# kisasexypantera94/hpfw

Measured on AMD Instinct MI355X. Metric: hashprints/sec (index) + Hamming matches/sec (search), 30 s@44.1 kHz clips, higher is better.
Workload: dtype f32 (transforms, dB) + int8 digits / int64 sums (projection); 1 GPU; configs[1]: 1000 x 30 s synthetic 44.1 kHz PCM16 clips per GPU, hashprint extraction only (CQT + dB + projection + bit pack), inputs resident in HBM; clips_per_gpu=1000, hashprints_per_clip=2320, parallelism=clips sharded over 1 GPU(s), no collective on this path

## Files before the change

hpfw_amd/csrc/extract.hip:

```cpp
#include "handle.h"

int pass_clips(hpfw_gpu *h, const DevPlan *dp, int64_t n_clips)
{
    const hpfw::HostPlan &p = dp->hp;
    size_t per_clip = (size_t)121 * p.c * 4 + (size_t)64 * std::max(p.n_frames, 1) * 4;
    if (p.bluestein)
        per_clip += 2 * hpfw::bz_plane_bytes(dp->bz, 1) + (size_t)(p.kmax - p.kmin) * 8;
    else
        per_clip += (size_t)hpfw::z_floats_per_clip(p.hq, p.n2) * 4 + (size_t)p.n1 * p.q2w * 8;
    size_t work = 0;
    for (const hpfw::CqClassDev &cd : dp->cls) work = std::max(work, hpfw::cq_big_work_bytes(cd, 1));
    per_clip += work;
    const int64_t fit = std::max<int64_t>(1, (int64_t)(((size_t)24 << 30) / per_clip));
    const int64_t cap = std::min<int64_t>(h->batch, fit), n = std::max<int64_t>(n_clips, 1);
    const int64_t passes = (n + cap - 1) / cap;
    return (int)((n + passes - 1) / passes);
}

int ensure_ws(hpfw_gpu *h, const DevPlan *dp, int nb, int ns)
{
    const hpfw::HostPlan &p = dp->hp;
    size_t work = 0;
    for (const hpfw::CqClassDev &cd : dp->cls) work = std::max(work, hpfw::cq_big_work_bytes(cd, nb));
    if (work) {
        int rc = ensure(h->d_cqwork, work);
        if (rc) return rc;
    }
    const size_t planar = p.bluestein ? hpfw::bz_plane_bytes(dp->bz, nb) : 0;
    const size_t need[7] = {p.bluestein ? planar : (size_t)nb * hpfw::z_floats_per_clip(p.hq, p.n2) * 4,
                            p.bluestein ? (size_t)nb * (p.kmax - p.kmin) * 8 : (size_t)nb * p.n1 * p.q2w * 8,
                            (size_t)ns * 121 * p.c * 4, (size_t)ns * 64 * (size_t)std::max(p.n_frames, 1) * 4,
                            (size_t)ns * 121 * hpfw::kCqMaxWaves * 4,
                            0, planar};
    for (int i = 0; i < 7; ++i) {
        int rc = ensure(h->ws[i], need[i], h);
        if (rc) return rc;
    }
    return ensure(h->d_clipmax, (size_t)ns * 4, h);
}

namespace {
int ensure_side_streams(hpfw_gpu *h)
{
    if (h->cq_join[hpfw_gpu::kCqSide - 1]) return HPFW_OK;
    bool ok = h->cq_fork.create() == hipSuccess;
    for (int k = 0; k < hpfw_gpu::kCqSide && ok; ++k) ok = h->cq_side[k].create() == hipSuccess && h->cq_join[k].create() == hipSuccess;
    return ok ? HPFW_OK : fail(HPFW_E_HIP, "side streams");
}

class Fanout {
public:
    Fanout(hpfw_gpu *h, hipStream_t s) : h_(h), s_(s) {}
    Fanout(const Fanout &) = delete;
    Fanout &operator=(const Fanout &) = delete;
    ~Fanout()
    {
        for (int k = 0; k < hpfw_gpu::kCqSide; ++k) {
            if (!(used_ >> k & 1u)) continue;
            hipStream_t side = h_->cq_side[k].get();
            hipEvent_t join = h_->cq_join[k].get();
            if (report(h_, hipEventRecord(join, side), "side stream join") || report(h_, hipStreamWaitEvent(s_, join, 0), "side stream join"))
                (void)hipStreamSynchronize(side);
        }
    }
    int fork(int n)
    {
        int rc = ensure_side_streams(h_);
        if (rc) return rc;
        HIP_TRY(hipEventRecord(h_->cq_fork.get(), s_));
        for (int k = 0; k < n; ++k) HIP_TRY(hipStreamWaitEvent(h_->cq_side[k].get(), h_->cq_fork.get(), 0));
        return 0;
    }
    hipStream_t lane(int k)
    {
        if (k == 0) return s_;
        used_ |= 1u << (k - 1);
        return h_->cq_side[k - 1].get();
    }

private:
    hpfw_gpu *h_;
    hipStream_t s_;
    unsigned used_ = 0;
};

#if defined(HPFW_ROWS_SNAP) || defined(HPFW_ROWS_STAMPS)
hpfw::cf *g_rows_snap = nullptr;
#endif

int run_forward(hpfw_gpu *h, DevPlan *dp, const int16_t *d_pcm, int nb, hpfw::cf *x, hipStream_t s)
{
    const hpfw::HostPlan &p = dp->hp;
    float *yp = h->ws[0].as<float>();
    int rc;
    if (p.bluestein) {
        float *other = h->ws[6].as<float>();
        if (h->bz_chunk > 0 && nb >= 6 * h->bz_chunk) {
            const int lanes = h->fwd_streams;
            Fanout fan(h, s);
            if (lanes > 1 && (rc = fan.fork(lanes - 1))) return rc;
            const int64_t region = (int64_t)(hpfw::bz_plane_bytes(dp->bz, h->bz_chunk) / sizeof(float));
            int i = 0;
            for (int c0 = 0; c0 < nb; c0 += h->bz_chunk, ++i) {
                const int nc = std::min(nb - c0, h->bz_chunk);
                const int lane = i % lanes;
                hipStream_t st = fan.lane(lane);
                float *ya = yp + lane * region, *yb = other + lane * region;
                {
                    Timed t(h, K_COLS, st);
                    hpfw::launch_bz_cols_first(dp->bz, d_pcm + (int64_t)c0 * p.n, p.n, nc, ya, st);
                }
                {
                    Timed t(h, K_ROWS, st);
                    hpfw::launch_bz_rows_both(dp->rows, dp->bz, ya, nc, yb, st);
                }
                {
                    Timed t(h, K_COLS, st);
                    hpfw::launch_bz_cols_last(dp->bz, yb, nc, x + (int64_t)c0 * dp->cq.xclip, st);
                }
            }
            return check_launch("bz_chunks");
        }
        {
            Timed t(h, K_COLS, s);
            hpfw::launch_bz_cols_first(dp->bz, d_pcm, p.n, nb, yp, s);
        }
        if ((rc = check_launch("bz_cols"))) return rc;
        {
            Timed t(h, K_ROWS, s);
            hpfw::launch_bz_rows_both(dp->rows, dp->bz, yp, nb, other, s);
        }
        if ((rc = check_launch("bz_rows"))) return rc;
        {
            Timed t(h, K_COLS, s);
            hpfw::launch_bz_cols_last(dp->bz, other, nb, x, s);
        }
        return check_launch("bz_cols");
    }
    Timed span(h, K_FWD, s);
    hpfw::ColsQArgs cols = dp->cols;
    cols.variant = h->cols_variant;
    if (h->fwd_chunk > 0 && nb >= 6 * h->fwd_chunk) {
        const int lanes = h->fwd_streams;
        Fanout fan(h, s);
        if (lanes > 1 && (rc = fan.fork(lanes - 1))) return rc;
        const int64_t region = (int64_t)h->fwd_chunk * dp->rows_out.zclip;
        int i = 0;
        for (int c0 = 0; c0 < nb; c0 += h->fwd_chunk, ++i) {
            const int nc = std::min(nb - c0, h->fwd_chunk);
            const int lane = i % lanes;
            hipStream_t st = fan.lane(lane);
            float *zr = yp + lane * region;
            {
                Timed t(h, K_COLS, st);
                hpfw::launch_fwd_cols_q(cols, d_pcm + (int64_t)c0 * p.n, p.n, nc, zr, st);
            }
            {
                Timed t(h, K_ROWS, st);
                hpfw::launch_fwd_rows2(dp->rows, dp->rows_out, zr, nc, x + (int64_t)c0 * dp->rows_out.n1 * dp->rows_out.q2w, st);
            }
        }
        return check_launch("fwd_chunks");
    }
    {
        Timed t(h, K_COLS, s);
        hpfw::launch_fwd_cols_q(cols, d_pcm, p.n, nb, yp, s);
    }
    if ((rc = check_launch("fwd_cols"))) return rc;
    {
        Timed t(h, K_ROWS, s);
#if defined(HPFW_ROWS_SNAP)
        dp->rows.snap = g_rows_snap;
#endif
#if defined(HPFW_ROWS_STAMPS)
        dp->rows.stamps = reinterpret_cast<long long *>(g_rows_snap);
#endif
        hpfw::launch_fwd_rows2(dp->rows, dp->rows_out, yp, nb, x, s);
    }
    return check_launch("fwd_rows");
}
}

int run_front(hpfw_gpu *h, DevPlan *dp, const int16_t *d_pcm, int nb, int slot, bool finish_db, hipStream_t s)
{
    using hpfw::cf;
    const hpfw::HostPlan &p = dp->hp;
    cf *x = h->ws[1].as<cf>();
    float *mag = h->ws[2].as<float>() + (size_t)slot * 121 * p.c;
    float *mm = h->ws[4].as<float>() + (size_t)slot * 121 * hpfw::kCqMaxWaves;
    float *clipmax = h->d_clipmax.as<float>() + slot;
    int rc;
    if ((rc = run_forward(h, dp, d_pcm, nb, x, s))) return rc;
    {
        Timed t(h, K_CQ, s);
        int n_lds = 0;
        for (const hpfw::CqClassDev &cd : dp->cls) n_lds += cd.outer ? 0 : 1;
        const bool fork = h->cq_concurrent && n_lds > 1 && nb >= 4;
        Fanout fan(h, s);
        if (fork && (rc = fan.fork(hpfw_gpu::kCqSide))) return rc;
        int turn = 0;
        for (size_t ci = dp->cls.size(); ci-- > 0;) {
            const hpfw::CqClassDev &cd = dp->cls[ci];
            if (cd.outer) {
                hpfw::launch_cq_big_class(dp->cq, cd, x, nb, h->d_cqwork.as<cf>(), mag, mm, h->db_fast ? hpfw::kDbFast : hpfw::kDbSpec, s);
                continue;
            }
            const int lane = fork ? turn++ % (hpfw_gpu::kCqSide + 1) : 0;
            hpfw::launch_cq_class(dp->cq, cd, x, nb, mag, mm, h->db_fast ? hpfw::kDbFast : hpfw::kDbSpec, fan.lane(lane));
        }
        if ((rc = check_launch("cq_chirpz"))) return rc;
    }
    {
        Timed t(h, K_DB, s);
        hpfw::launch_clipmax(mm, clipmax, nb, s);
        if (finish_db) hpfw::launch_db_finish(mag, clipmax, nb, (int64_t)121 * p.c, s);
    }
    return check_launch("db");
}

int q_split(hpfw_gpu *h, int n_shifts, int64_t n_clips, int64_t c, hpfw::QSplit *qs, const hpfw::QSplit **use)
{
    *use = nullptr;
    if (n_shifts || h->q_products != 6 || !h->projection) return 0;
    const int64_t tiles = hpfw::project_q_tiles(n_clips, c);
    if (tiles <= 0) return 0;
    if (int rc = ensure(h->d_q_split, hpfw::project_q_split_bytes(tiles), h)) return rc;
    *qs = {h->d_q_thr.as<int32_t>(), h->d_q_split.get()};
    *use = qs;
    return 0;
}

namespace {
int run_back(hpfw_gpu *h, DevPlan *dp, const void *images, int n_shifts, int ns, uint64_t *d_hp, hipStream_t s)
{
    const hpfw::HostPlan &p = dp->hp;
    const float *sdb = h->ws[2].as<float>();
    int rc;
    if (h->projection) {
        hpfw::QSplit qs;
        const hpfw::QSplit *split;
        if ((rc = q_split(h, n_shifts, ns, p.c, &qs, &split))) return rc;
        {
            Timed t(h, K_PROJECT, s);
            hpfw::launch_hashprints_q(images, n_shifts, sdb, h->d_clipmax.as<float>(), ns, p.c, d_hp, nullptr, s, split);
        }
        if (split) h->q_last_tiles = hpfw::project_q_tiles(ns, p.c);
        return check_launch("project");
    }
    float *proj = h->ws[3].as<float>();
    {
        Timed t(h, K_PROJECT, s);
        hpfw::launch_project(h->d_fpack.as<float>(), sdb, h->d_clipmax.as<float>(), ns, p.c, proj, s);
    }
    if ((rc = check_launch("project"))) return rc;
    {
        Timed t(h, K_PACK, s);
        hpfw::launch_pack(proj, ns, p.n_frames, d_hp, s);
    }
    return check_launch("delta_pack");
}

constexpr int kBackBatch = 1024;

int check_filters(const hpfw_gpu *h) { return h->has_filters ? 0 : fail(HPFW_E_NOFILTERS, "no filters: call hpfw_gpu_set_filters or hpfw_gpu_learn_filters first"); }

int check_shifts(const int32_t *shifts, int n_shifts)
{
    if (!shifts || n_shifts < 1 || n_shifts > hpfw::kMaxShifts) return fail(HPFW_E_INVALID, "shifts: 1 to 64 values");
    for (int i = 0; i < n_shifts; ++i) {
        if (shifts[i] < -(hpfw::kBins - 1) || shifts[i] > hpfw::kBins - 1) return fail(HPFW_E_INVALID, "shifts: |s| <= 120");
        for (int j = 0; j < i; ++j)
            if (shifts[j] == shifts[i]) return fail(HPFW_E_INVALID, "shifts: values must be distinct");
    }
    return 0;
}

int shift_images(hpfw_gpu *h, const int32_t *shifts, int n_shifts, hipStream_t s)
{
    std::vector<int32_t> want(shifts, shifts + n_shifts);
    if (want == h->shift_images_of) return 0;
    h->shift_images_of.clear();
    int rc;
    if ((rc = ensure(h->d_shift_images, (size_t)n_shifts * hpfw::project_q_image_bytes()))) return rc;
    hpfw::ShiftList sl{n_shifts, {}};
    for (int i = 0; i < n_shifts; ++i) sl.s[i] = shifts[i];
    hpfw::launch_shift_filter_images(h->d_fq_image.get(), sl, h->d_shift_images.get(), s);
    if ((rc = check_launch("shift_filter_images"))) return rc;
    h->shift_images_of = std::move(want);
    return 0;
}

int check_transposed(hpfw_gpu *h, const int32_t *shifts, int n_shifts)
{
    int rc;
    if ((rc = check_shifts(shifts, n_shifts))) return rc;
    if (!h) return fail(HPFW_E_INVALID, "null handle");
    if (!h->projection) return fail(HPFW_E_INVALID, "transposed extraction needs projection mode 1 (fixed point)");
    if ((rc = check_filters(h))) return rc;
    return 0;
}

int hashprints_from_db(hpfw_gpu *h, const float *d_db, int64_t n_clips, int64_t c, const int32_t *shifts, int n_shifts, uint64_t *d_hp,
                       hipStream_t s)
{
    const int64_t nf = c - (hpfw::kCtx - 1), nhp = nf - hpfw::kLag;
    HIP_TRY(hipSetDevice(h->device));
    return ordered_call(h, s, [&] {
        int rc;
        if (n_shifts && (rc = shift_images(h, shifts, n_shifts, s))) return rc;
        const void *images = n_shifts ? h->d_shift_images.get() : h->d_fq_image.get();
        const int nbmax = 256;
        if (!h->projection && (rc = ensure(h->ws[3], (size_t)nbmax * 64 * (size_t)nf * 4))) return rc;
        hpfw::QSplit qs;
        const hpfw::QSplit *split;
        if ((rc = q_split(h, n_shifts, std::min<int64_t>(nbmax, n_clips), c, &qs, &split))) return rc;
        for (int64_t c0 = 0; c0 < n_clips; c0 += nbmax) {
            const int nb = (int)std::min<int64_t>(nbmax, n_clips - c0);
            if (h->projection) {
                Timed t(h, K_PROJECT, s);
                hpfw::launch_hashprints_q(images, n_shifts, d_db + c0 * 121 * c, nullptr, nb, (int)c, d_hp + c0 * std::max(n_shifts, 1) * nhp,
                                          nullptr, s, split);
                if (split) h->q_last_tiles = hpfw::project_q_tiles(nb, c);
            } else {
                hpfw::launch_project(h->d_fpack.as<float>(), d_db + c0 * 121 * c, nullptr, nb, (int)c, h->ws[3].as<float>(), s);
                hpfw::launch_pack(h->ws[3].as<float>(), nb, (int)nf, d_hp + c0 * nhp, s);
            }
            if ((rc = check_launch("project"))) return rc;
        }
        return 0;
    });
}

constexpr size_t kTempoBudget = (size_t)256 << 20;

int check_tempos(const float *tempos, int n_tempos, int n_shifts)
{
    if (!tempos || n_tempos < 1 || n_tempos > hpfw::kMaxTempos) return fail(HPFW_E_INVALID, "tempos: 1 to 64 values");
    for (int i = 0; i < n_tempos; ++i) {
        if (!(tempos[i] >= 0.5f && tempos[i] <= 2.0f)) return fail(HPFW_E_INVALID, "tempos: finite values in [0.5, 2]");
        for (int j = 0; j < i; ++j)
            if (hpfw::tempo_step(tempos[j]) == hpfw::tempo_step(tempos[i]))
                return fail(HPFW_E_INVALID, "tempos: values must have distinct steps rint(65536 / tempo)");
    }
    if ((int64_t)n_tempos * std::max(n_shifts, 1) > hpfw::kMaxShifts) return fail(HPFW_E_INVALID, "tempos x shifts: at most 64 variants");
    return 0;
}

int check_tempo_call(hpfw_gpu *h, const float *tempos, int n_tempos, const int32_t *shifts, int n_shifts, hpfw::TempoList *tl)
{
    int rc;
    if ((rc = check_tempos(tempos, n_tempos, n_shifts))) return rc;
    if ((shifts || n_shifts) && (rc = check_shifts(shifts, n_shifts))) return rc;
    if (!h) return fail(HPFW_E_INVALID, "null handle");
    if (!h->projection) return fail(HPFW_E_INVALID, "tempo extraction needs projection mode 1 (fixed point)");
    if ((rc = check_filters(h))) return rc;
    tl->n = n_tempos;
    for (int i = 0; i < n_tempos; ++i) tl->step[i] = hpfw::tempo_step(tempos[i]);
    return 0;
}

int64_t tempo_common_columns(int64_t c, const hpfw::TempoList &tl)
{
    int64_t ct = INT64_MAX;
    for (int i = 0; i < tl.n; ++i) ct = std::min(ct, hpfw::tempo_columns(c, tl.step[i]));
    return ct;
}

int tempo_back(hpfw_gpu *h, const void *images, int n_shifts, const float *d_db, int64_t nb, int64_t c, const hpfw::TempoList &tl,
               int64_t ct, uint64_t *d_hp, hipStream_t s)
{
    const int64_t per_pair = (int64_t)std::max(n_shifts, 1) * (ct - (hpfw::kCtx - 1) - hpfw::kLag);
    const size_t pair_bytes = (size_t)hpfw::kBins * ct * 4;
    const int64_t pairs = std::max<int64_t>(1, (int64_t)(kTempoBudget / pair_bytes));
    const int64_t cb = pairs >= tl.n ? std::min<int64_t>(pairs / tl.n, nb) : 1;
    const int tb = pairs >= tl.n ? tl.n : (int)pairs;
    int rc;
    if ((rc = ensure(h->d_tempo, (size_t)cb * tb * pair_bytes, h))) return rc;
    float *scaled = h->d_tempo.as<float>();
    for (int64_t c0 = 0; c0 < nb; c0 += cb) {
        const int nc = (int)std::min(cb, nb - c0);
        for (int j0 = 0; j0 < tl.n; j0 += tb) {
            hpfw::TempoList sub{std::min(tb, tl.n - j0), {}};
            for (int j = 0; j < sub.n; ++j) sub.step[j] = tl.step[j0 + j];
            hpfw::launch_tempo_scale(d_db + c0 * hpfw::kBins * c, nc, c, sub, ct, scaled, s);
            if ((rc = check_launch("tempo_scale"))) return rc;
            {
                Timed t(h, K_PROJECT, s);
                hpfw::launch_hashprints_q(images, n_shifts, scaled, nullptr, nc * sub.n, (int)ct, d_hp + (c0 * tl.n + j0) * per_pair, nullptr, s);
            }
            if ((rc = check_launch("project"))) return rc;
        }
    }
    return 0;
}

int extract_tempo_pcm16(hpfw_gpu *h, const int16_t *d_pcm, int64_t n_samples, int64_t n_clips, const float *tempos, int n_tempos,
                        const int32_t *shifts, int n_shifts, uint64_t *d_hp, void *stream)
{
    hpfw::TempoList tl;
    int rc = check_tempo_call(h, tempos, n_tempos, shifts, n_shifts, &tl);
    if (rc) return rc;
    if (!d_pcm || !d_hp || n_clips < 0) return fail(HPFW_E_INVALID, "bad argument");
    HIP_TRY(hipSetDevice(h->device));
    DevPlan *dp;
    if ((rc = get_plan(h, n_samples, &dp))) return rc;
    const int64_t c = dp->hp.c, ct = tempo_common_columns(c, tl);
    if (ct - (hpfw::kCtx - 1) - hpfw::kLag < 1) return fail(HPFW_E_UNSUPPORTED, "clip too short to yield a hashprint at the slowest tempo");
    if (n_clips == 0) return 0;
    const int64_t per_clip = (int64_t)tl.n * std::max(n_shifts, 1) * (ct - (hpfw::kCtx - 1) - hpfw::kLag);
    hipStream_t s = (hipStream_t)stream;
    return ordered_call(h, s, [&] {
        if (n_shifts && (rc = shift_images(h, shifts, n_shifts, s))) return rc;
        const void *images = n_shifts ? h->d_shift_images.get() : h->d_fq_image.get();
        const int nbmax = pass_clips(h, dp, n_clips);
        if ((rc = ensure_ws(h, dp, nbmax, nbmax))) return rc;
        for (int64_t c0 = 0; c0 < n_clips; c0 += nbmax) {
            const int nb = (int)std::min<int64_t>(nbmax, n_clips - c0);
            if ((rc = run_front(h, dp, d_pcm + c0 * n_samples, nb, 0, true, s))) return rc;
            if ((rc = tempo_back(h, images, n_shifts, h->ws[2].as<float>(), nb, c, tl, ct, d_hp + c0 * per_clip, s))) return rc;
        }
        return 0;
    });
}

int extract_pcm16(hpfw_gpu *h, const int16_t *d_pcm, int64_t n_samples, int64_t n_clips, const int32_t *shifts, int n_shifts,
                  uint64_t *d_hp, void *stream)
{
    if (!h || !d_pcm || !d_hp || n_clips < 0) return fail(HPFW_E_INVALID, "bad argument");
    if (int rc = check_filters(h)) return rc;
    HIP_TRY(hipSetDevice(h->device));
    DevPlan *dp;
    int rc = get_plan(h, n_samples, &dp);
    if (rc) return rc;
    if (dp->hp.n_hp <= 0) return fail(HPFW_E_UNSUPPORTED, "clip too short to yield a hashprint");
    hipStream_t s = (hipStream_t)stream;
    return ordered_call(h, s, [&] {
        if (n_shifts && (rc = shift_images(h, shifts, n_shifts, s))) return rc;
        const void *images = n_shifts ? h->d_shift_images.get() : h->d_fq_image.get();
        const int nbmax = pass_clips(h, dp, n_clips);
        const int nsmax = (int)std::min<int64_t>(std::max(kBackBatch, nbmax), std::max<int64_t>(n_clips, 1));
        if ((rc = ensure_ws(h, dp, nbmax, nsmax))) return rc;
        for (int64_t s0 = 0; s0 < n_clips; s0 += nsmax) {
            const int ns = (int)std::min<int64_t>(nsmax, n_clips - s0);
            for (int c0 = 0; c0 < ns; c0 += nbmax) {
                const int nb = std::min(nbmax, ns - c0);
                if ((rc = run_front(h, dp, d_pcm + (s0 + c0) * n_samples, nb, c0, false, s))) return rc;
            }
            if ((rc = run_back(h, dp, images, n_shifts, ns, d_hp + s0 * std::max(n_shifts, 1) * dp->hp.n_hp, s))) return rc;
        }
        return 0;
    });
}

template <class Device>
int staged_pcm16_host(hpfw_gpu *h, const int16_t *pcm, int64_t n_samples, int64_t n_clips, int64_t per_clip, uint64_t *hp,
                      Device device)
{
    int rc;
    const int64_t chunk = std::min<int64_t>(n_clips, std::max<int64_t>(1, (192ll << 20) / (n_samples * 2)));
    if ((rc = ensure(h->stage_hp, (size_t)n_clips * std::max<int64_t>(per_clip, 1) * 8))) return rc;
    for (int b = 0; b < 2; ++b) {
        if (b == 1 && chunk >= n_clips) break;
        if ((rc = ensure(h->stage_pcm[b], (size_t)chunk * n_samples * 2))) return rc;
    }
    if (!h->stage_consumed[1]) {
        HIP_TRY(h->stage_copy.create());
        HIP_TRY(h->stage_comp.create());
        for (int b = 0; b < 2; ++b) {
            HIP_TRY(h->stage_copied[b].create());
            HIP_TRY(h->stage_consumed[b].create());
        }
    }
    hipStream_t s_copy = h->stage_copy.get(), s_comp = h->stage_comp.get();
    uint64_t *d_hp = h->stage_hp.as<uint64_t>();
    int64_t ci = 0;
    for (int64_t c0 = 0; !rc && c0 < n_clips; c0 += chunk, ++ci) {
        const int b = (int)(ci & 1);
        const int64_t cnt = std::min(chunk, n_clips - c0);
        int16_t *d_pcm = h->stage_pcm[b].as<int16_t>();
        hipEvent_t copied = h->stage_copied[b].get(), consumed = h->stage_consumed[b].get();
        if (ci >= 2 && hipStreamWaitEvent(s_copy, consumed, 0) != hipSuccess) rc = fail(HPFW_E_HIP, "event wait failed");
        if (!rc && hipMemcpyAsync(d_pcm, pcm + c0 * n_samples, (size_t)cnt * n_samples * 2, hipMemcpyHostToDevice, s_copy) !=
                       hipSuccess)
            rc = fail(HPFW_E_HIP, "H2D copy failed");
        if (!rc && (hipEventRecord(copied, s_copy) != hipSuccess || hipStreamWaitEvent(s_comp, copied, 0) != hipSuccess))
            rc = fail(HPFW_E_HIP, "event record failed");
        if (!rc) rc = device(d_pcm, cnt, d_hp + c0 * per_clip, s_comp);
        if (!rc && hipEventRecord(consumed, s_comp) != hipSuccess) rc = fail(HPFW_E_HIP, "event record failed");
    }
    if (hipStreamSynchronize(s_copy) != hipSuccess && !rc) rc = fail(HPFW_E_HIP, "H2D copy failed");
    if (!rc && hipMemcpyAsync(hp, d_hp, (size_t)n_clips * per_clip * 8, hipMemcpyDeviceToHost, s_comp) != hipSuccess)
        rc = fail(HPFW_E_HIP, "D2H copy failed");
    if (hipStreamSynchronize(s_comp) != hipSuccess && !rc) rc = fail(HPFW_E_HIP, "kernel execution failed");
    return rc;
}
}

extern "C" {

int hpfw_gpu_hashprints_from_db(hpfw_gpu *h, const float *d_db, int64_t n_clips, int64_t c, uint64_t *d_hp, void *stream)
{
    if (!h || !d_db || !d_hp) return fail(HPFW_E_INVALID, "null argument");
    if (int rc = check_filters(h)) return rc;
    if (c - (hpfw::kCtx - 1) - hpfw::kLag <= 0) return 0;
    return hashprints_from_db(h, d_db, n_clips, c, nullptr, 0, d_hp, (hipStream_t)stream);
}

int hpfw_gpu_debug_q_products(hpfw_gpu *h, int64_t *tiles, int64_t *listed, int64_t *redone)
{
    if (!h || !tiles || !listed || !redone) return fail(HPFW_E_INVALID, "null argument");
    *tiles = *listed = *redone = 0;
    if (h->q_products != 6 || h->q_last_tiles <= 0) return 0;
    HIP_TRY(hipSetDevice(h->device));
    HIP_TRY(hipDeviceSynchronize());
    std::vector<uint32_t> counts((size_t)h->q_last_tiles);
    HIP_TRY(hipMemcpy(counts.data(), h->d_q_split.get(), counts.size() * 4, hipMemcpyDeviceToHost));
    *tiles = h->q_last_tiles;
    for (uint32_t v : counts) {
        if (v == 0xffffffffu) *redone += 1;
        else *listed += v;
    }
    return 0;
}

int hpfw_gpu_stage_delta_q(hpfw_gpu *h, const float *d_db, int64_t n_clips, int64_t c, int64_t *d_delta, uint64_t *d_hp, void *stream)
{
    if (!h || !d_db || !d_delta) return fail(HPFW_E_INVALID, "null argument");
    if (int rc = check_filters(h)) return rc;
    const int64_t nhp = c - (hpfw::kCtx - 1) - hpfw::kLag;
    if (nhp <= 0 || n_clips <= 0) return 0;
    if (n_clips > 65535) return fail(HPFW_E_INVALID, "at most 65535 clips per call");
    HIP_TRY(hipSetDevice(h->device));
    hipStream_t s = (hipStream_t)stream;
    return ordered_call(h, s, [&] {
        uint64_t *hp = d_hp;
        if (!hp) {
            if (int rc = ensure(h->ws[3], (size_t)n_clips * (size_t)nhp * 8)) return rc;
            hp = h->ws[3].as<uint64_t>();
        }
        hpfw::launch_hashprints_q(h->d_fq_image.get(), 0, d_db, nullptr, (int)n_clips, (int)c, hp, (long long *)d_delta, s);
        return check_launch("project");
    });
}

int hpfw_gpu_hashprints_from_db_transposed(hpfw_gpu *h, const float *d_db, int64_t n_clips, int64_t c, const int32_t *shifts,
                                           int n_shifts, uint64_t *d_hp, void *stream)
{
    int rc = check_transposed(h, shifts, n_shifts);
    if (rc) return rc;
    if (!d_db || !d_hp || n_clips < 0) return fail(HPFW_E_INVALID, "bad argument");
    if (c - (hpfw::kCtx - 1) - hpfw::kLag <= 0 || n_clips == 0) return 0;
    return hashprints_from_db(h, d_db, n_clips, c, shifts, n_shifts, d_hp, (hipStream_t)stream);
}

int hpfw_gpu_extract_pcm16(hpfw_gpu *h, const int16_t *d_pcm, int64_t n_samples, int64_t n_clips,
                           uint64_t *d_hp, void *stream)
{
    return extract_pcm16(h, d_pcm, n_samples, n_clips, nullptr, 0, d_hp, stream);
}

int hpfw_gpu_extract_transposed_pcm16(hpfw_gpu *h, const int16_t *d_pcm, int64_t n_samples, int64_t n_clips, const int32_t *shifts,
                                      int n_shifts, uint64_t *d_hp, void *stream)
{
    if (int rc = check_transposed(h, shifts, n_shifts)) return rc;
    return extract_pcm16(h, d_pcm, n_samples, n_clips, shifts, n_shifts, d_hp, stream);
}

static int extract_pcm16_host(hpfw_gpu *h, const int16_t *pcm, int64_t n_samples, int64_t n_clips, const int32_t *shifts, int n_shifts,
                              uint64_t *hp)
{
    if (!h || !pcm || !hp || n_clips < 0) return fail(HPFW_E_INVALID, "bad argument");
    HIP_TRY(hipSetDevice(h->device));
    hpfw_geometry g;
    int rc = hpfw_gpu_geometry(h, n_samples, &g);
    if (rc) return rc;
    if (n_clips == 0) return 0;
    return staged_pcm16_host(h, pcm, n_samples, n_clips, std::max(n_shifts, 1) * g.n_hp, hp,
                             [&](const int16_t *d_pcm, int64_t cnt, uint64_t *d_hp, hipStream_t st) {
                                 return extract_pcm16(h, d_pcm, n_samples, cnt, shifts, n_shifts, d_hp, st);
                             });
}

int hpfw_gpu_extract_pcm16_host(hpfw_gpu *h, const int16_t *pcm, int64_t n_samples, int64_t n_clips, uint64_t *hp)
{
    return extract_pcm16_host(h, pcm, n_samples, n_clips, nullptr, 0, hp);
}

int hpfw_gpu_extract_transposed_pcm16_host(hpfw_gpu *h, const int16_t *pcm, int64_t n_samples, int64_t n_clips, const int32_t *shifts,
                                           int n_shifts, uint64_t *hp)
{
    if (int rc = check_transposed(h, shifts, n_shifts)) return rc;
    return extract_pcm16_host(h, pcm, n_samples, n_clips, shifts, n_shifts, hp);
}

int hpfw_gpu_tempo_columns(int64_t c, const float *tempos, int n_tempos, int64_t *c_out)
{
    if (int rc = check_tempos(tempos, n_tempos, 0)) return rc;
    if (c < 1 || !c_out) return fail(HPFW_E_INVALID, "bad argument");
    hpfw::TempoList tl{n_tempos, {}};
// ... 404 lines not shown
```

hpfw_amd/csrc/handle.h:

```cpp
#pragma once
#include <hip/hip_runtime.h>

#include <algorithm>
#include <cstdio>
#include <cstdlib>
#include <cstring>
#include <condition_variable>
#include <chrono>
#include <map>
#include <memory>
#include <mutex>
#include <set>
#include <string>
#include <vector>

#include "../../include/hpfw_gpu.h"
#include "combiner.h"
#include "hip_owned.h"
#include "kernels.h"
#include "legacy_internal.h"
#include "plan.h"

using hpfw::DevBuf, hpfw::Event, hpfw::HostBuf, hpfw::Stream;

int fail(int code, const std::string &msg);

#define HIP_TRY(expr)                                                                                   \
    do {                                                                                                \
        hipError_t e_ = (expr);                                                                         \
        if (e_ != hipSuccess)                                                                           \
            return fail(HPFW_E_HIP, std::string(#expr) + ": " + hipGetErrorString(e_));                 \
    } while (0)

struct DevPlan {
    hpfw_gpu *owner = nullptr;
    std::vector<DevBuf> blocks;
    char *cur = nullptr;
    size_t left = 0;
    char *chunk_base = nullptr;
    std::vector<char> stage;
    std::vector<std::pair<size_t, size_t>> staged;
    hpfw::HostPlan hp;
    hpfw::ColsQArgs cols;
    hpfw::Rows2Out rows_out;
    hpfw::RowsArgs rows;
    hpfw::BzArgs bz;
    hpfw::CqPlanDev cq;
    std::vector<hpfw::CqClassDev> cls;
    size_t bytes = 0;
    uint64_t last_use = 0;
    ~DevPlan();
};

struct PlanTiming;

enum KernelKind { K_ROWS = 0, K_COLS, K_CQ, K_DB, K_PROJECT, K_PACK, K_SCAN, K_TOPK, K_PAIRS, K_FWD, K_COUNT };

struct TimedLaunch {
    int kind;
    Event a, b;
};

struct CallStatus {
    int rc = 0;
    std::string msg;
};

struct hpfw_gpu {
    int device = 0;
    bool has_filters = false;
    std::vector<float> filters;
    DevBuf d_fpack;
    DevBuf d_fq_image;
    DevBuf d_q_thr, d_q_split;
    int q_products = 6;
    int64_t q_last_tiles = 0;
    int projection = 1;
    struct PlanCache {
        PlanCache();
        ~PlanCache();
        std::multimap<size_t, DevBuf> dev_pool;
        size_t dev_pool_bytes = 0;
        std::map<int64_t, std::unique_ptr<DevPlan>> plans;
        std::mutex host_mtx;
        std::condition_variable host_cv;
        std::map<int64_t, std::unique_ptr<hpfw::HostPlan>> host_ready;
        std::set<int64_t> host_seen;
        size_t plan_bytes = 0;
        uint64_t plan_clock = 0;
        uint64_t idle_clock = 0;
        std::unique_ptr<PlanTiming> plan_timing;
        Stream plan_stream;
        HostBuf pin_ring;
        size_t pin_off = 0;
        Event plan_ev;
        bool plan_ev_pending = false;
    } cache;
    unsigned conventions = 0;
    int batch = 256;
    DevBuf ws[7];
    struct Index {
        DevBuf d_db;
        std::vector<int64_t> db_off{0};
        DevBuf d_db_off;
        bool db_off_dirty = true;
        uint32_t clip_base = 0;
        DevBuf d_best, d_q_off;
        DevBuf d_qa;
        DevBuf d_gk;
        DevBuf d_topk_scratch;
        DevBuf d_shift_hits;
        DevBuf d_ov_tab, d_ov_exclude;
        DevBuf d_within_tab, d_within_q, d_within_out;
        DevBuf d_sj_tab, d_sj_rows, d_sj_pairs;
        DevBuf d_sj_x_off;
        DevBuf d_votes_ws, d_votes_tab;
        DevBuf d_dtw_q_off, d_dtw_pairs, d_dtw_bnd, d_dtw_hits, d_dtw_top, d_dtw_choices;
        DevBuf d_local_top, d_local_flag;
        DevBuf d_stage, d_moves;
        std::vector<hpfw_index_move> moves;
        Event moves_ev;
        bool moves_pending = false;
    } index;
    struct Learn {
        DevBuf d_cov;
        DevBuf d_cov_ws;
        DevBuf d_cov_tiles;
        int64_t cov_files = 0;
        std::map<std::vector<int>, DevBuf> cfg_fpack;
        DevBuf d_cfg_proj;
        struct CfgCov {
            DevBuf d_accum;
            DevBuf d_tiles;
            int64_t clips = 0;
        };
        std::map<std::vector<int>, CfgCov> cfg_cov;
        DevBuf d_cfg_cov_ws;
    } learn;
    struct Mel {
        bool ready = false;
        hpfw::HostPlan plan;
        hpfw::RowsArgs rows;
        const float *d_win = nullptr, *d_cpack = nullptr;
        std::vector<DevBuf> owned;
        DevBuf d_work, d_small;
    } mel;
    DevBuf d_cqwork;
    static constexpr int kCqSide = 4;
    Stream cq_side[kCqSide];
    Event cq_fork, cq_join[kCqSide];
    int cq_concurrent = 1;
    int fwd_chunk = 16, fwd_streams = 2;
    int cols_variant = 0;
    unsigned prune = 1;
    bool db_fast = true;
    int bz_chunk = 32;
    DevBuf stage_pcm[2];
    DevBuf stage_hp;
    Stream stage_copy, stage_comp;
    Event stage_copied[2], stage_consumed[2];
    DevBuf d_clipmax;
    Event order_ev;
    hipStream_t order_stream = nullptr;
    enum { kOrderNone, kOrderEvent, kOrderSync } order = kOrderNone;
    CallStatus call;
    Event ev0, ev1;
    unsigned timing_mask = 0;
    std::vector<TimedLaunch> timed;
    std::vector<std::pair<Event, Event>> ev_pool;
    float k_ms[K_COUNT] = {0};
    int k_launches[K_COUNT] = {0};
    std::unique_ptr<hpfw::Combiner> combiner;
    struct Xcorr {
        DevBuf d_tab, d_r;
    } xcorr;
    struct Resample {
        struct Table {
            int32_t L = 0, M = 0, T = 0;
            DevBuf d_taps;
        };
        std::map<int, Table> tables;
        DevBuf in, out;
    } rs;
    struct Warp {
        DevBuf d_taps, d_tracks;
    } warp;
    DevBuf d_shift_images;
    std::vector<int32_t> shift_images_of;
    DevBuf d_tempo;
    DevBuf d_windows;
};

int ensure(DevBuf &b, size_t need, hpfw_gpu *pool_owner = nullptr);

inline int report(hpfw_gpu *h, hipError_t e, const char *what)
{
    if (e != hipSuccess && !h->call.rc) h->call = {HPFW_E_HIP, std::string(what) + ": " + hipGetErrorString(e)};
    return e != hipSuccess;
}

template <class Body>
int ordered_call(hpfw_gpu *h, hipStream_t s, Body &&body)
{
    if (h->order_stream != s) {
        if (h->order == hpfw_gpu::kOrderEvent) HIP_TRY(hipStreamWaitEvent(s, h->order_ev.get(), 0));
        if (h->order == hpfw_gpu::kOrderSync) HIP_TRY(hipStreamSynchronize(h->order_stream));
    }
    if (h->cache.plan_ev_pending) {
        HIP_TRY(hipStreamWaitEvent(s, h->cache.plan_ev.get(), 0));
        h->cache.plan_ev_pending = false;
    }
    CallStatus outer = std::exchange(h->call, CallStatus{});
    int rc = body();
    const hipError_t recorded = hipEventRecord(h->order_ev.get(), s);
    h->order_stream = s;
    h->order = recorded == hipSuccess ? hpfw_gpu::kOrderEvent : hpfw_gpu::kOrderSync;
    CallStatus mine = std::exchange(h->call, std::move(outer));
    if (!rc && mine.rc) rc = fail(mine.rc, mine.msg);
    if (!rc && recorded != hipSuccess) rc = fail(HPFW_E_HIP, std::string("hipEventRecord: ") + hipGetErrorString(recorded));
    return rc;
}

struct Timed {
    hpfw_gpu *h;
    int kind;
    hipStream_t s;
    bool on = false;
    Event a, b;
    Timed(hpfw_gpu *h_, int kind_, hipStream_t s_) : h(h_), kind(kind_), s(s_)
    {
        if (!((h->timing_mask >> kind) & 1u)) return;
        if (h->ev_pool.empty()) {
            if (report(h, a.create(hipEventDefault), "timing event") || report(h, b.create(hipEventDefault), "timing event")) return;
        } else {
            a = std::move(h->ev_pool.back().first);
            b = std::move(h->ev_pool.back().second);
            h->ev_pool.pop_back();
        }
        on = !report(h, hipEventRecord(a.get(), s), "timing event record");
    }
    ~Timed()
    {
        if (on && !report(h, hipEventRecord(b.get(), s), "timing event record")) h->timed.push_back({kind, std::move(a), std::move(b)});
    }
};

inline int check_launch(const char *what)
{
    hipError_t e = hipGetLastError();
    if (e != hipSuccess) return fail(HPFW_E_HIP, std::string("launch of ") + what + ": " + hipGetErrorString(e));
    return 0;
}

struct HostTrip {
    int rc = 0;
    std::vector<std::pair<DevBuf, void *>> bufs;
    template <class T>
    T *take(size_t bytes, const void *src = nullptr, int fill = -1, void *dst = nullptr)
    {
        DevBuf &b = bufs.emplace_back(DevBuf(), dst).first;
        if (!rc && b.alloc(bytes) != hipSuccess) rc = fail(HPFW_E_NOMEM, "hipMalloc failed");
        if (!rc && ((src && hipMemcpy(b.get(), src, bytes, hipMemcpyHostToDevice) != hipSuccess) ||
                    (fill >= 0 && hipMemset(b.get(), fill, bytes) != hipSuccess)))
            rc = fail(HPFW_E_HIP, "H2D copy failed");
        return b.as<T>();
    }
    template <class Call>
    int run(bool wait, Call call)
    {
        if (!rc) rc = call();
        if (!rc && wait && hipDeviceSynchronize() != hipSuccess) rc = fail(HPFW_E_HIP, "kernel execution failed");
        for (auto &[b, dst] : bufs)
            if (!rc && dst && hipMemcpy(dst, b.get(), b.capacity(), hipMemcpyDeviceToHost) != hipSuccess) rc = fail(HPFW_E_HIP, "D2H copy failed");
        return rc;
    }
};

template <class Q, class Hit, class Device>
int search_round_trip_scored(const Q *q_hp, const int64_t *q_off, int64_t n_sets, int64_t n_out, Hit *out, int64_t n_stats,
                             hpfw_dist_stats *stats, Device device)
{
    const int64_t total = q_off[n_sets] - q_off[0];
    if (total < 0) return fail(HPFW_E_INVALID, "q_off must be non-decreasing");
    if (total && !q_hp) return fail(HPFW_E_INVALID, "null queries");
    std::vector<int64_t> rel((size_t)n_sets + 1);
    for (int64_t i = 0; i <= n_sets; ++i) rel[(size_t)i] = q_off[i] - q_off[0];
    HostTrip t;
    const Q *d_q = t.take<Q>((size_t)std::max<int64_t>(total, 1) * sizeof(Q), total ? q_hp + q_off[0] : nullptr);
    Hit *d_out = t.take<Hit>((size_t)n_out * sizeof(Hit), nullptr, -1, out);
    hpfw_dist_stats *d_stats = n_stats ? t.take<hpfw_dist_stats>((size_t)n_stats * sizeof(hpfw_dist_stats), nullptr, -1, stats) : nullptr;
    return t.run(true, [&] { return device(d_q, rel.data(), d_out, d_stats); });
}

template <class Q, class Hit, class Device>
int search_round_trip(const Q *q_hp, const int64_t *q_off, int64_t n_sets, int64_t n_out, Hit *out, Device device)
{
    return search_round_trip_scored(q_hp, q_off, n_sets, n_out, out, 0, nullptr,
                                    [&](const Q *d_q, const int64_t *rel, Hit *d_out, hpfw_dist_stats *) { return device(d_q, rel, d_out); });
}

inline int upload_db_off(hpfw_gpu *h, hipStream_t s)
{
    if (!h->index.db_off_dirty) return 0;
    if (int rc = ensure(h->index.d_db_off, h->index.db_off.size() * 8)) return rc;
    HIP_TRY(hipMemcpyAsync(h->index.d_db_off.get(), h->index.db_off.data(), h->index.db_off.size() * 8, hipMemcpyHostToDevice, s));
    HIP_TRY(hipStreamSynchronize(s));
    h->index.db_off_dirty = false;
    return 0;
}

inline int64_t index_longest_clip(const hpfw_gpu *h)
{
    int64_t n_max = 0;
    for (size_t i = 0; i + 1 < h->index.db_off.size(); ++i) n_max = std::max(n_max, h->index.db_off[i + 1] - h->index.db_off[i]);
    return n_max;
}

inline int64_t overlap_splits(int64_t chunks, int64_t pairs, const char *env_name)
{
    if (const char *e = std::getenv(env_name)) return std::min<int64_t>(std::max(std::atoi(e), 1), 64);
    return std::min<int64_t>({chunks, (2048 + pairs - 1) / pairs, 64});
}

int get_plan(hpfw_gpu *h, int64_t n, DevPlan **out);
hipError_t init_plans(hpfw_gpu *h);
void clear_plans(hpfw_gpu *h);
int q_split(hpfw_gpu *h, int n_shifts, int64_t n_clips, int64_t c, hpfw::QSplit *qs, const hpfw::QSplit **use);
int pass_clips(hpfw_gpu *h, const DevPlan *dp, int64_t n_clips);
int ensure_ws(hpfw_gpu *h, const DevPlan *dp, int nb, int ns);
int run_front(hpfw_gpu *h, DevPlan *dp, const int16_t *d_pcm, int nb, int slot, bool finish_db, hipStream_t s);
int rs_table(hpfw_gpu *h, int rate, hpfw_gpu::Resample::Table **out);
```

hpfw_amd/csrc/handle.hip:

```cpp
#include "handle.h"

namespace {
thread_local std::string g_err;

const char *const kKernelNames[K_COUNT] = {"fwd_rows", "fwd_cols", "cq_chirpz", "db",
                                           "project_mfma", "delta_pack", "hamming_scan", "topk", "pcm_pairs", "fwd_span"};
}

int fail(int code, const std::string &msg)
{
    g_err = msg;
    return code;
}

extern "C" {

const char *hpfw_gpu_last_error(void) { return g_err.c_str(); }
void hpfw_internal_set_error(const char *msg) { g_err = msg ? msg : ""; }
const char *hpfw_gpu_version(void) { return "hpfw-gpu 0.1 (gfx950)"; }

int hpfw_gpu_create(int device, hpfw_gpu **out)
{
    if (!out) return fail(HPFW_E_INVALID, "out is NULL");
    *out = nullptr;
    int n = 0;
    HIP_TRY(hipGetDeviceCount(&n));
    if (device < 0 || device >= n) return fail(HPFW_E_INVALID, "no such device");
    HIP_TRY(hipSetDevice(device));
    auto h = std::make_unique<hpfw_gpu>();
    h->device = device;
    if (std::getenv("HPFW_CQ_SERIAL")) h->cq_concurrent = 0;
    if (const char *e = std::getenv("HPFW_FWD_CHUNK")) h->fwd_chunk = std::max(0, atoi(e));
    if (const char *e = std::getenv("HPFW_BZ_CHUNK")) h->bz_chunk = std::max(0, atoi(e));
    if (const char *e = std::getenv("HPFW_COLS_VARIANT")) h->cols_variant = atoi(e);
    if (const char *e = std::getenv("HPFW_PRUNE")) h->prune = (unsigned)std::strtoul(e, nullptr, 0);
    if (const char *e = std::getenv("HPFW_Q_PRODUCTS")) h->q_products = atoi(e) == 9 ? 9 : 6;
    if (const char *e = std::getenv("HPFW_DB_TERM")) h->db_fast = std::strcmp(e, "spec") != 0;
    if (const char *e = std::getenv("HPFW_FWD_STREAMS")) h->fwd_streams = std::min(hpfw_gpu::kCqSide + 1, std::max(1, atoi(e)));
    if (const char *e = std::getenv("HPFW_PROJECTION"))
        h->projection = std::strcmp(e, "f32") == 0 ? 0 : 1;
    if (h->ev0.create(hipEventDefault) != hipSuccess || h->ev1.create(hipEventDefault) != hipSuccess || h->order_ev.create() != hipSuccess ||
        init_plans(h.get()) != hipSuccess)
        return fail(HPFW_E_HIP, "hipEventCreate failed");
    *out = h.release();
    return 0;
}

int hpfw_gpu_device(const hpfw_gpu *h) { return h ? h->device : -1; }

void hpfw_gpu_destroy(hpfw_gpu *h)
{
    if (!h) return;
    (void)hipSetDevice(h->device);
    (void)hipDeviceSynchronize();
    delete h;
}

int hpfw_gpu_set_filters(hpfw_gpu *h, const float *f)
{
    if (!h || !f) return fail(HPFW_E_INVALID, "null argument");
    HIP_TRY(hipSetDevice(h->device));
    std::vector<float> packed((size_t)hpfw::kFilters * hpfw::kFrame);
    hpfw::pack_filters_for_mfma(f, packed.data());
    if (!h->d_fpack) HIP_TRY(h->d_fpack.alloc(packed.size() * 4));
    HIP_TRY(hipMemcpy(h->d_fpack.get(), packed.data(), packed.size() * 4, hipMemcpyHostToDevice));
    std::vector<int8_t> image;
    std::vector<int32_t> thr;
    hpfw::pack_filters_q(f, image, &thr);
    if (!h->d_fq_image) HIP_TRY(h->d_fq_image.alloc(image.size()));
    HIP_TRY(hipMemcpy(h->d_fq_image.get(), image.data(), image.size(), hipMemcpyHostToDevice));
    if (!h->d_q_thr) HIP_TRY(h->d_q_thr.alloc(thr.size() * 4));
    HIP_TRY(hipMemcpy(h->d_q_thr.get(), thr.data(), thr.size() * 4, hipMemcpyHostToDevice));
    h->shift_images_of.clear();
    h->filters.assign(f, f + (size_t)hpfw::kFilters * hpfw::kFrame);
    h->has_filters = true;
    return 0;
}

int hpfw_gpu_get_filters(hpfw_gpu *h, float *out)
{
    if (!h || !out) return fail(HPFW_E_INVALID, "null argument");
    if (!h->has_filters) return fail(HPFW_E_NOFILTERS, "no filters: call hpfw_gpu_set_filters or hpfw_gpu_learn_filters first");
    std::memcpy(out, h->filters.data(), h->filters.size() * sizeof(float));
    return 0;
}

int hpfw_gpu_set_projection(hpfw_gpu *h, int mode)
{
    if (!h || (mode != 0 && mode != 1)) return fail(HPFW_E_INVALID, "projection mode must be 0 (f32 chain) or 1 (fixed point)");
    h->projection = mode;
    return 0;
}

int hpfw_gpu_get_projection(hpfw_gpu *h) { return h ? h->projection : -1; }

int hpfw_gpu_set_conventions(hpfw_gpu *h, unsigned flags)
{
    if (!h || flags > hpfw::kConvAll) return fail(HPFW_E_INVALID, "unknown convention flag");
    HIP_TRY(hipSetDevice(h->device));
    if (flags != h->conventions) {
        HIP_TRY(hipDeviceSynchronize());
        clear_plans(h);
    }
    h->conventions = flags;
    return 0;
}

int hpfw_gpu_set_batch(hpfw_gpu *h, int clips)
{
    if (!h || clips < 0 || clips > 4096) return fail(HPFW_E_INVALID, "batch out of range");
    h->batch = clips == 0 ? 256 : clips;
    return 0;
}

int hpfw_gpu_timer_start(hpfw_gpu *h, void *stream)
{
    if (!h) return fail(HPFW_E_INVALID, "null handle");
    HIP_TRY(hipEventRecord(h->ev0.get(), (hipStream_t)stream));
    return 0;
}

int hpfw_gpu_timer_stop(hpfw_gpu *h, void *stream, float *ms)
{
    if (!h || !ms) return fail(HPFW_E_INVALID, "null argument");
    HIP_TRY(hipEventRecord(h->ev1.get(), (hipStream_t)stream));
    HIP_TRY(hipEventSynchronize(h->ev1.get()));
    HIP_TRY(hipEventElapsedTime(ms, h->ev0.get(), h->ev1.get()));
    return 0;
}

int hpfw_gpu_set_kernel_timing(hpfw_gpu *h, int mask)
{
    if (!h) return fail(HPFW_E_INVALID, "null handle");
    h->timing_mask = (unsigned)mask;
    for (TimedLaunch &t : h->timed) h->ev_pool.emplace_back(std::move(t.a), std::move(t.b));
    h->timed.clear();
    std::memset(h->k_ms, 0, sizeof(h->k_ms));
    std::memset(h->k_launches, 0, sizeof(h->k_launches));
    return 0;
}

int hpfw_gpu_get_kernel_timing(hpfw_gpu *h, const char **names, float *ms, int *launches, int *n)
{
    if (!h || !names || !ms || !launches || !n) return fail(HPFW_E_INVALID, "null argument");
    for (const TimedLaunch &t : h->timed) {
        HIP_TRY(hipEventSynchronize(t.b.get()));
        float e = 0.0f;
        HIP_TRY(hipEventElapsedTime(&e, t.a.get(), t.b.get()));
        h->k_ms[t.kind] += e;
        h->k_launches[t.kind] += 1;
    }
    for (TimedLaunch &t : h->timed) h->ev_pool.emplace_back(std::move(t.a), std::move(t.b));
    h->timed.clear();
    const int cap = *n;
    int w = 0;
    for (int i = 0; i < K_COUNT && w < cap; ++i, ++w) {
        names[w] = kKernelNames[i];
        ms[w] = h->k_ms[i];
        launches[w] = h->k_launches[i];
    }
    *n = w;
    return 0;
}

}
```

Before: 291.3 million hashprints/s.

## Pipeline forward transform of next pass with CQ classes of current pass

Adds a pass-level software pipeline. The forward transform (cols+rows) for pass i+1 is queued into a second x buffer while the constant-Q class kernels for pass i run on side streams, with per-lane events providing cross-stream dependencies. This aims to hide the idle gaps between the forward and CQ stages across passes within a group. In exchange it doubles the x workspace, which shrinks the clips-per-pass fit, and adds event-wait overhead. It is enabled by default only when there are at least two passes and the last pass is large enough.

```diff
diff --git a/hpfw_amd/csrc/extract.hip b/hpfw_amd/csrc/extract.hip
--- a/hpfw_amd/csrc/extract.hip
+++ b/hpfw_amd/csrc/extract.hip
@@ -1,4 +1,6 @@
 #include "handle.h"
+
+#include <optional>
 
 int pass_clips(hpfw_gpu *h, const DevPlan *dp, int64_t n_clips)
 {
@@ -7,7 +9,7 @@
     if (p.bluestein)
         per_clip += 2 * hpfw::bz_plane_bytes(dp->bz, 1) + (size_t)(p.kmax - p.kmin) * 8;
     else
-        per_clip += (size_t)hpfw::z_floats_per_clip(p.hq, p.n2) * 4 + (size_t)p.n1 * p.q2w * 8;
+        per_clip += (size_t)hpfw::z_floats_per_clip(p.hq, p.n2) * 4 + (size_t)p.n1 * p.q2w * 8 * (h->pass_pipeline ? 2 : 1);
     size_t work = 0;
     for (const hpfw::CqClassDev &cd : dp->cls) work = std::max(work, hpfw::cq_big_work_bytes(cd, 1));
     per_clip += work;
@@ -17,7 +19,7 @@
     return (int)((n + passes - 1) / passes);
 }
 
-int ensure_ws(hpfw_gpu *h, const DevPlan *dp, int nb, int ns)
+int ensure_ws(hpfw_gpu *h, const DevPlan *dp, int nb, int ns, int x_bufs)
 {
     const hpfw::HostPlan &p = dp->hp;
     size_t work = 0;
@@ -28,7 +30,7 @@
     }
     const size_t planar = p.bluestein ? hpfw::bz_plane_bytes(dp->bz, nb) : 0;
     const size_t need[7] = {p.bluestein ? planar : (size_t)nb * hpfw::z_floats_per_clip(p.hq, p.n2) * 4,
-                            p.bluestein ? (size_t)nb * (p.kmax - p.kmin) * 8 : (size_t)nb * p.n1 * p.q2w * 8,
+                            p.bluestein ? (size_t)nb * (p.kmax - p.kmin) * 8 : (size_t)x_bufs * nb * p.n1 * p.q2w * 8,
                             (size_t)ns * 121 * p.c * 4, (size_t)ns * 64 * (size_t)std::max(p.n_frames, 1) * 4,
                             (size_t)ns * 121 * hpfw::kCqMaxWaves * 4,
                             0, planar};
@@ -44,6 +46,8 @@
 {
     if (h->cq_join[hpfw_gpu::kCqSide - 1]) return HPFW_OK;
     bool ok = h->cq_fork.create() == hipSuccess;
+    for (int b = 0; b < 2 && ok; ++b)
+        for (int k = 0; k <= hpfw_gpu::kCqSide && ok; ++k) ok = h->pp_fwd[b][k].create() == hipSuccess && h->pp_cq[b][k].create() == hipSuccess;
     for (int k = 0; k < hpfw_gpu::kCqSide && ok; ++k) ok = h->cq_side[k].create() == hipSuccess && h->cq_join[k].create() == hipSuccess;
     return ok ? HPFW_OK : fail(HPFW_E_HIP, "side streams");
 }
@@ -87,6 +91,32 @@
 #if defined(HPFW_ROWS_SNAP) || defined(HPFW_ROWS_STAMPS)
 hpfw::cf *g_rows_snap = nullptr;
 #endif
+
+void queue_fwd_chunks(hpfw_gpu *h, DevPlan *dp, const int16_t *d_pcm, int nb, hpfw::cf *x, Fanout &fan,
+                      const std::vector<int> *turns = nullptr)
+{
+    const hpfw::HostPlan &p = dp->hp;
+    hpfw::ColsQArgs cols = dp->cols;
+    cols.variant = h->cols_variant;
+    float *yp = h->ws[0].as<float>();
+    const int lanes = h->fwd_streams;
+    const int64_t region = (int64_t)h->fwd_chunk * dp->rows_out.zclip;
+    int i = 0;
+    for (int c0 = 0; c0 < nb; c0 += h->fwd_chunk, ++i) {
+        const int nc = std::min(nb - c0, h->fwd_chunk);
+        const int lane = turns ? (*turns)[i % turns->size()] : i % lanes;
+        hipStream_t st = fan.lane(lane);
+        float *zr = yp + lane * region;
+        {
+            Timed t(h, K_COLS, st);
+            hpfw::launch_fwd_cols_q(cols, d_pcm + (int64_t)c0 * p.n, p.n, nc, zr, st);
+        }
+        {
+            Timed t(h, K_ROWS, st);
+            hpfw::launch_fwd_rows2(dp->rows, dp->rows_out, zr, nc, x + (int64_t)c0 * dp->rows_out.n1 * dp->rows_out.q2w, st);
+        }
+    }
+}
 
 int run_forward(hpfw_gpu *h, DevPlan *dp, const int16_t *d_pcm, int nb, hpfw::cf *x, hipStream_t s)
 {
@@ -144,22 +174,7 @@
         const int lanes = h->fwd_streams;
         Fanout fan(h, s);
         if (lanes > 1 && (rc = fan.fork(lanes - 1))) return rc;
-        const int64_t region = (int64_t)h->fwd_chunk * dp->rows_out.zclip;
-        int i = 0;
-        for (int c0 = 0; c0 < nb; c0 += h->fwd_chunk, ++i) {
-            const int nc = std::min(nb - c0, h->fwd_chunk);
-            const int lane = i % lanes;
-            hipStream_t st = fan.lane(lane);
-            float *zr = yp + lane * region;
-            {
-                Timed t(h, K_COLS, st);
-                hpfw::launch_fwd_cols_q(cols, d_pcm + (int64_t)c0 * p.n, p.n, nc, zr, st);
-            }
-            {
-                Timed t(h, K_ROWS, st);
-                hpfw::launch_fwd_rows2(dp->rows, dp->rows_out, zr, nc, x + (int64_t)c0 * dp->rows_out.n1 * dp->rows_out.q2w, st);
-            }
-        }
+        queue_fwd_chunks(h, dp, d_pcm, nb, x, fan);
         return check_launch("fwd_chunks");
     }
     {
@@ -262,6 +277,78 @@
 
 constexpr int kBackBatch = 1024;
 
+bool group_pipelines(const hpfw_gpu *h, const DevPlan *dp, int ns, int nbmax)
+{
+    constexpr unsigned kept = 1u << K_PROJECT | 1u << K_FWD;
+    if (!h->pass_pipeline || dp->hp.bluestein || !h->cq_concurrent || h->fwd_chunk <= 0 || (h->timing_mask & ~kept)) return false;
+    for (const hpfw::CqClassDev &cd : dp->cls)
+        if (cd.outer) return false;
+    const int passes = (ns + nbmax - 1) / nbmax, last = ns - (passes - 1) * nbmax;
+    return passes >= 2 && last >= 6 * h->fwd_chunk;
+}
+
+int run_group_pipelined(hpfw_gpu *h, DevPlan *dp, const int16_t *d_pcm, int ns, int nbmax, hipStream_t s)
+{
+    using hpfw::cf;
+    const hpfw::HostPlan &p = dp->hp;
+    constexpr int kLanes = hpfw_gpu::kCqSide + 1;
+    const int passes = (ns + nbmax - 1) / nbmax;
+    const int64_t xbuf = (int64_t)nbmax * p.n1 * p.q2w;
+    const int db = h->db_fast ? hpfw::kDbFast : hpfw::kDbSpec;
+    std::vector<int> turns = h->pp_turns, lane_of(dp->cls.size());
+    if (turns.empty())
+        for (int k = 0; k < h->fwd_streams; ++k) turns.push_back(k);
+    unsigned fwd_lanes = 0, cq_lanes = 0;
+    for (int k : turns) fwd_lanes |= 1u << k;
+    const int fl = h->fwd_streams;
+    for (size_t ci = dp->cls.size(), i = 0; ci-- > 0; ++i) {
+        if (!h->pp_class_lane.empty()) lane_of[ci] = h->pp_class_lane[std::min(i, h->pp_class_lane.size() - 1)];
+        else lane_of[ci] = i == 0 ? std::min(fl, kLanes - 1) : i == 1 ? fl - 1 : 0;
+        cq_lanes |= 1u << lane_of[ci];
+    }
+    int rc;
+    {
+        Fanout fan(h, s);
+        if ((rc = fan.fork(hpfw_gpu::kCqSide))) return rc;
+        std::optional<Timed> span;
+        auto forward = [&](int pass) -> int {
+            const int c0 = pass * nbmax, nb = std::min(nbmax, ns - c0), b = pass & 1;
+            span.emplace(h, K_FWD, s);
+            if (pass >= 2)
+                for (int k = 0; k < kLanes; ++k)
+                    for (int j = 0; j < kLanes; ++j)
+                        if ((fwd_lanes >> k & 1u) && (cq_lanes >> j & 1u) && j != k) HIP_TRY(hipStreamWaitEvent(fan.lane(k), h->pp_cq[b][j].get(), 0));
+            queue_fwd_chunks(h, dp, d_pcm + (int64_t)c0 * p.n, nb, h->ws[1].as<cf>() + b * xbuf, fan, &turns);
+            for (int k = 0; k < kLanes; ++k)
+                if (fwd_lanes >> k & 1u) HIP_TRY(hipEventRecord(h->pp_fwd[b][k].get(), fan.lane(k)));
+            return check_launch("fwd_chunks");
+        };
+        auto classes = [&](int pass) -> int {
+            const int c0 = pass * nbmax, nb = std::min(nbmax, ns - c0), b = pass & 1;
+            const bool timed = span && span->on;
+            for (int j = 0; j < kLanes; ++j)
+                if ((cq_lanes >> j & 1u) || (j == 0 && timed))
+                    for (int k = 0; k < kLanes; ++k)
+                        if ((fwd_lanes >> k & 1u) && k != j) HIP_TRY(hipStreamWaitEvent(fan.lane(j), h->pp_fwd[b][k].get(), 0));
+            span.reset();
+            for (size_t ci = dp->cls.size(); ci-- > 0;)
+                hpfw::launch_cq_class(dp->cq, dp->cls[ci], h->ws[1].as<cf>() + b * xbuf, nb, h->ws[2].as<float>() + (size_t)c0 * 121 * p.c,
+                                      h->ws[4].as<float>() + (size_t)c0 * 121 * hpfw::kCqMaxWaves, db, fan.lane(lane_of[ci]));
+            if (pass + 2 < passes)
+                for (int j = 0; j < kLanes; ++j)
+                    if (cq_lanes >> j & 1u) HIP_TRY(hipEventRecord(h->pp_cq[b][j].get(), fan.lane(j)));
+            return check_launch("cq_chirpz");
+        };
+        if ((rc = forward(0))) return rc;
+        for (int pass = 0; pass < passes; ++pass) {
+            if ((rc = classes(pass))) return rc;
+            if (pass + 1 < passes && (rc = forward(pass + 1))) return rc;
+        }
+    }
+    hpfw::launch_clipmax(h->ws[4].as<float>(), h->d_clipmax.as<float>(), ns, s);
+    return check_launch("db");
+}
+
 int check_filters(const hpfw_gpu *h) { return h->has_filters ? 0 : fail(HPFW_E_NOFILTERS, "no filters: call hpfw_gpu_set_filters or hpfw_gpu_learn_filters first"); }
 
 int check_shifts(const int32_t *shifts, int n_shifts)
@@ -439,12 +526,17 @@
         const void *images = n_shifts ? h->d_shift_images.get() : h->d_fq_image.get();
         const int nbmax = pass_clips(h, dp, n_clips);
         const int nsmax = (int)std::min<int64_t>(std::max(kBackBatch, nbmax), std::max<int64_t>(n_clips, 1));
-        if ((rc = ensure_ws(h, dp, nbmax, nsmax))) return rc;
+        const bool pipelined = group_pipelines(h, dp, (int)std::min<int64_t>(nsmax, n_clips), nbmax);
+        if ((rc = ensure_ws(h, dp, nbmax, nsmax, pipelined ? 2 : 1))) return rc;
         for (int64_t s0 = 0; s0 < n_clips; s0 += nsmax) {
             const int ns = (int)std::min<int64_t>(nsmax, n_clips - s0);
-            for (int c0 = 0; c0 < ns; c0 += nbmax) {
-                const int nb = std::min(nbmax, ns - c0);
-                if ((rc = run_front(h, dp, d_pcm + (s0 + c0) * n_samples, nb, c0, false, s))) return rc;
+            if (pipelined && group_pipelines(h, dp, ns, nbmax)) {
+                if ((rc = run_group_pipelined(h, dp, d_pcm + s0 * n_samples, ns, nbmax, s))) return rc;
+            } else {
+                for (int c0 = 0; c0 < ns; c0 += nbmax) {
+                    const int nb = std::min(nbmax, ns - c0);
+                    if ((rc = run_front(h, dp, d_pcm + (s0 + c0) * n_samples, nb, c0, false, s))) return rc;
+                }
             }
             if ((rc = run_back(h, dp, images, n_shifts, ns, d_hp + s0 * std::max(n_shifts, 1) * dp->hp.n_hp, s))) return rc;
         }
diff --git a/hpfw_amd/csrc/handle.h b/hpfw_amd/csrc/handle.h
--- a/hpfw_amd/csrc/handle.h
+++ b/hpfw_amd/csrc/handle.h
@@ -150,6 +150,9 @@
     Stream cq_side[kCqSide];
     Event cq_fork, cq_join[kCqSide];
     int cq_concurrent = 1;
+    Event pp_fwd[2][kCqSide + 1], pp_cq[2][kCqSide + 1];
+    int pass_pipeline = 1;
+    std::vector<int> pp_class_lane, pp_turns;
     int fwd_chunk = 16, fwd_streams = 2;
     int cols_variant = 0;
     unsigned prune = 1;
@@ -327,6 +330,6 @@
 void clear_plans(hpfw_gpu *h);
 int q_split(hpfw_gpu *h, int n_shifts, int64_t n_clips, int64_t c, hpfw::QSplit *qs, const hpfw::QSplit **use);
 int pass_clips(hpfw_gpu *h, const DevPlan *dp, int64_t n_clips);
-int ensure_ws(hpfw_gpu *h, const DevPlan *dp, int nb, int ns);
+int ensure_ws(hpfw_gpu *h, const DevPlan *dp, int nb, int ns, int x_bufs = 1);
 int run_front(hpfw_gpu *h, DevPlan *dp, const int16_t *d_pcm, int nb, int slot, bool finish_db, hipStream_t s);
 int rs_table(hpfw_gpu *h, int rate, hpfw_gpu::Resample::Table **out);
diff --git a/hpfw_amd/csrc/handle.hip b/hpfw_amd/csrc/handle.hip
--- a/hpfw_amd/csrc/handle.hip
+++ b/hpfw_amd/csrc/handle.hip
@@ -31,6 +31,14 @@
     h->device = device;
     if (std::getenv("HPFW_CQ_SERIAL")) h->cq_concurrent = 0;
     if (const char *e = std::getenv("HPFW_FWD_CHUNK")) h->fwd_chunk = std::max(0, atoi(e));
+    if (const char *e = std::getenv("HPFW_PASS_PIPELINE")) h->pass_pipeline = atoi(e) != 0;
+    if (const char *e = std::getenv("HPFW_PASS_PLAN")) {
+        std::vector<int> *to = &h->pp_class_lane;
+        for (; *e; ++e) {
+            if (*e == ':') to = &h->pp_turns;
+            else if (*e >= '0' && *e <= '0' + hpfw_gpu::kCqSide) to->push_back(*e - '0');
+        }
+    }
     if (const char *e = std::getenv("HPFW_BZ_CHUNK")) h->bz_chunk = std::max(0, atoi(e));
     if (const char *e = std::getenv("HPFW_COLS_VARIANT")) h->cols_variant = atoi(e);
     if (const char *e = std::getenv("HPFW_PRUNE")) h->prune = (unsigned)std::strtoul(e, nullptr, 0);
```

New measurement: 296.4 million hashprints/s, median of 6. 1.8% higher.
